# ipo-lab/lqp_py

Hardware: AMD Instinct MI355X
Metric: QPs/sec forward+backward, batch=128 dz=500 tol=1e-5 (higher is better)
Workload: dtype f32; 1 GPU; BASELINE configs[2]: batch=128/GPU dz=500 m=1 box+equality QP, ADMM forward + fixed-point backward, eps 1e-5, scale+adaptive_rho defaults; global_batch=128, seeds=10 batches, seeds 0..9 per rank, cycled, iters=60, checks=4, launch_mode=3, sync=False, linsolve=spd, loop_workgroups_per_qp=2, parallelism=batch-sharded x1, rccl_world_size=1

## Files before the change

lqp_py_amd/csrc/lqp_amd.hip:

```cpp
#include "../../include/lqp_amd.h"
#include "lqp_boxqp.hpp"
#include "lqp_unroll.hpp"
#ifdef LQP_SPLIT_BUILD
#include "split/lqp_extern.inc"
#endif

#include <cstdio>
#include <cstdlib>
#include <cstring>
#include <algorithm>
#include <atomic>
#include <chrono>
#include <mutex>
#include <vector>
#include <string>
#include <unordered_map>

using namespace lqp;

namespace {

constexpr int kRing = 2048;
inline int max_rows(int dtype) { return dtype == LQP_F32 ? 4096 : 2048; }
constexpr size_t kAlign = 256;
// ... 1179 lines not shown
    SoloScope one_wg_lu;
    for (;;) {
        const Knobs k = knobs();
        if (retry & 4) one_wg_lu.enter();
        FwdParams<T> P = L.P;
        FwdPlan<T> plan;
        int rc = plan_forward(P, ctl, retry, k, d, plan);
        if (rc) return rc;
        int n_launch = 0;
        rc = enqueue_prologue(st, P, plan, n_launch);
        if (rc) return rc;
        const Attempt a = plan.up_front ? run_planned(st, P, plan, ctl, stats, n_launch) : run_chunked(st, P, plan, ctl, stats, n_launch);
        switch (a.why) {
        case GU_NONE: return a.status;
        case GU_NOT_SPD: retry |= 1; break;
        case GU_LU_TIMEOUT: one_wg_lu.enter(); break;
        case GU_SEG_TIMEOUT: retry |= 2; break;
        case GU_SHARED_TIMEOUT: retry |= 4; break;
        }
    }
}

template <typename T>
size_t carve_backward(void* ws, int B, int n, int m, BwdParams<T>& P) {
    P.B = B; P.n = n; P.m = m; P.N = n + m;
    P.Np = round_up(P.N, LQP_NB); P.K = P.Np / LQP_NB;
    Carver c(ws);
    P.info = c.take<int>(B);
    P.piv = c.take<int>((size_t)B * P.Np);
    P.dest = c.take<int>((size_t)B * P.Np);
    P.rhs = c.take<T>((size_t)B * P.Np);
    P.rhs2 = c.take<T>((size_t)B * P.Np);
    P.bsc = c.take<T>((size_t)B * P.Np);
    P.fidx = c.take<int>((size_t)B * n);
    P.nred = c.take<int>(B);
    P.M = c.take<T>((size_t)B * P.Np * P.Np);
    P.packed = c.take<T>((size_t)B * packed_blocks(P.K) * LQP_BLK);
    return c.off + kAlign;
}

template <typename T>
int backward_impl(hipStream_t st, int B, int n, int m, const void* g, const void* x, const void* u, const void* lams,
                  const void* nus, const void* Q, const void* A, const void* lb, const void* ub, int rho_mode,
                  double rho_value, const void* rho_in, void* dQ, void* dp, void* dA, void* db, void* dlb, void* dub,
                  int32_t* fail_index, void* ws, size_t ws_bytes, int linsolve, void* host_report, const int kkt = 0,
                  int phase = 0) {
    const Knobs k = knobs();
    BwdParams<T> P;
    memset(&P, 0, sizeof(P));
    P.kkt = kkt ? 1 : 0;
    const bool reported = (linsolve & LQP_BWD_REPORTED) != 0;
    linsolve &= ~LQP_BWD_REPORTED;
    if (linsolve & LQP_BWD_PREFACTORED) { linsolve &= ~LQP_BWD_PREFACTORED; if (phase == 0 && !kkt) phase = 2; }
    P.host_report = (int*)host_report;
    bool reset_pending = P.host_report != nullptr;
    P.early_report = k.bwd_early != 0 ? 1 : 0;
    const size_t need = carve_backward<T>(ws, B, n, m, P);
    if (ws_bytes < need) return LQP_ERR_WORKSPACE;
    if (!k.bwd_equil) P.bsc = nullptr;
    P.g = (const T*)g; P.x = (const T*)x; P.u = (const T*)u; P.lams = (const T*)lams; P.nus = (const T*)nus;
    P.Q = (const T*)Q; P.A = (const T*)A; P.lb = (const T*)lb; P.ub = (const T*)ub; P.rho_in = (const T*)rho_in;
    P.rho_value = (T)rho_value; P.rho_mode = rho_mode;
    P.dQ = (T*)dQ; P.dp = (T*)dp; P.dA = (T*)dA; P.db = (T*)db; P.dlb = (T*)dlb; P.dub = (T*)dub;
    P.dbg = g_lu_dbg;
    P.reduced = (k.bwd_full && !kkt) ? 0 : 1;
    const int* nvec = P.reduced ? P.nred : nullptr;
    bool chol = false;
    if constexpr (sizeof(T) == 4) {
        chol = P.reduced && linsolve == 2 && k.bwd_chol && round_up(n, LQP_NB) / LQP_NB <= SPD_BIGK &&
               m <= SPD_MAXM && bwd_chol_lds_bytes(n, m, m >= 3 ? 4 : 2) <= 160 * 1024;
    }
    const bool lu_phases = !chol && P.reduced && !kkt;
    if (!chol && !lu_phases) {
        if (phase == 1) return LQP_ERR_UNSUPPORTED;
        phase = 0;
    }
    P.phase = phase;
    P.reported = (reported && phase == 2 && P.host_report && P.early_report) ? 1 : 0;
    if (reset_pending && !P.reported) report_reset(P.host_report, B);
    reset_pending = false;
    if constexpr (sizeof(T) == 4) {
        if (chol) {
            P.chol = 1;
            if (phase != 2) {
                const int lds = (2 * round_up(n, 8) + LQP_NW + 8 + round_up(n, 64) + 64) * 4;
                ProfScope ps(st, PC_BWD_BUILD);
                const int split = B <= 128 ? 2 : 1;
                hipLaunchKernelGGL(k_bwd_build_chol<>, dim3(B, split), dim3(LQP_NT), lds, st, P);
            }
            const bool nr4 = m >= 3;
            const int lds = bwd_chol_lds_bytes(n, m, nr4 ? 4 : 2);
            {
                const int Kmax = round_up(n, LQP_NB) / LQP_NB;
                P.la_maxk = !k.bwd_lookahead ? 0 : (Kmax < SPD_MAXK ? Kmax : SPD_MAXK - 1);
            }
            auto chol_fn = nr4 ? k_bwd_chol_solve<4> : k_bwd_chol_solve<0>;
#if LQP_PIV_MFMA
            if (k.spd_f16 != 0 && k.bwd_f16 != 0) chol_fn = nr4 ? k_bwd_chol_solve<4, true> : k_bwd_chol_solve<0, true>;
#endif
            int r2 = ensure_lds((const void*)chol_fn, lds);
            if (r2) return r2;
            ProfScope ps(st, PC_BWD_CHOL);
            hipLaunchKernelGGL(chol_fn, dim3(B), dim3(LQP_NT), lds, st, P);
            if (phase == 1) return hipGetLastError() == hipSuccess ? LQP_OK : LQP_ERR_HIP;
        }
    }
    if (chol) {
    } else if (phase == 2) {
        ProfScope ps(st, PC_BWD_BUILD);
        hipLaunchKernelGGL(k_bwd_gather_rhs<T>, dim3(B), dim3(256), 0, st, P);
    } else if (P.reduced) {
        const int lds = (round_up(n, 8) + LQP_NW + 8) * 4;
        ProfScope ps(st, PC_BWD_BUILD);
        const int split = (B <= 128 && k.split2) ? 2 : 1;
        hipLaunchKernelGGL(k_bwd_build_reduced<T>, dim3(B, split), dim3(LQP_NT), lds, st, P);
    } else {
        ProfScope ps(st, PC_BWD_BUILD);
        hipLaunchKernelGGL(k_bwd_build<T>, dim3(B), dim3(LQP_NT), 0, st, P);
    }
    int rc = LQP_OK;
    if (!chol) {
        if (phase != 2) {
            rc = launch_lu(st, P.M, B, P.N, P.Np, (size_t)P.Np * P.Np, P.piv, P.Np, P.info, nullptr, nvec,
                           (unsigned long long*)P.packed, packed_blocks(P.K) * LQP_BLK * sizeof(T) / 8);
            if (rc) return rc;
            if (P.host_report && (phase == 1 || (P.early_report && fail_index))) {
                ProfScope ps(st, PC_MISC);
                hipLaunchKernelGGL(k_report_info<>, dim3((B + 255) / 256), dim3(256), 0, st, (const int*)P.info, P.host_report, B);
                P.lu_reported = 1;
            }
            rc = launch_pack<T>(st, B, P.M, P.N, P.Np, (size_t)P.Np * P.Np, P.piv, P.Np, P.packed, P.dest, nullptr, nvec);
            if (rc) return rc;
            if (phase == 1) return hipGetLastError() == hipSuccess ? LQP_OK : LQP_ERR_HIP;
        } else if (P.reported) P.lu_reported = 1;
        rc = launch_solve<T>(st, B, P.packed, P.N, P.dest, P.rhs, 1, (size_t)P.Np, 1, 0, nvec);
        if (rc) return rc;
        if (P.reduced && !kkt && k.bwd_refine) {
            const int lds = (round_up(n, 8) + round_up(m > 0 ? m : 1, 8)) * (int)sizeof(T) + round_up(n, 8) * 4;
            { ProfScope ps(st, PC_BWD_BUILD);
              hipLaunchKernelGGL(k_bwd_residual<T>, dim3(B, (B <= 128 && k.split2) ? 2 : 1), dim3(LQP_NT), lds, st, P); }
            rc = launch_solve<T>(st, B, P.packed, P.N, P.dest, P.rhs2, 1, (size_t)P.Np, 1, 0, nvec);
            if (rc) return rc;
            P.refine = 1;
        }
    }
    {
        const int lds = (2 * n + m + 8) * (int)sizeof(T);
        auto fn = k_bwd_epilogue<T>;
        rc = ensure_lds((const void*)fn, lds);
        if (rc) return rc;
        ProfScope ps(st, PC_BWD_EPILOGUE);
        const int slabs = (k.epi_slabs < 0 ? (B <= 128 ? 2 : 1) : k.epi_slabs);
        hipLaunchKernelGGL(fn, dim3(B, slabs), dim3(LQP_NT), lds, st, P);
    }
    if (hipGetLastError() != hipSuccess) return LQP_ERR_HIP;
    if (fail_index) {
        int fi = -1;
        if (P.host_report && k.sync_plan != 0) {
            rc = wait_report(st, P.host_report, B);
            if (rc) return rc;
            bool gave_up = false;
            for (int i = 0; i < B; ++i) {
                const int v = ((const volatile int*)P.host_report)[i];
                if (v != 0 && fi < 0) fi = i;
                gave_up = gave_up || v == -7;
            }
            rc = gave_up ? LQP_ERR_TIMEOUT : fi >= 0 ? LQP_ERR_SINGULAR : LQP_OK;
        } else
            rc = first_failure(st, P.info, B, &fi, P.host_report);
        if (rc == LQP_ERR_TIMEOUT && !chol && !t_single_wg_lu) {
            SingleWgLu only;
            return backward_impl<T>(st, B, n, m, g, x, u, lams, nus, Q, A, lb, ub, rho_mode, rho_value, rho_in, dQ, dp, dA,
                                    db, dlb, dub, fail_index, ws, ws_bytes, 1, host_report, kkt, 0);
        }
        if (rc == LQP_ERR_SINGULAR && chol)
            return backward_impl<T>(st, B, n, m, g, x, u, lams, nus, Q, A, lb, ub, rho_mode, rho_value, rho_in, dQ, dp, dA,
                                    db, dlb, dub, fail_index, ws, ws_bytes, 1, host_report, kkt, 0);
        *fail_index = fi;
// ... 754 lines not shown
```

lqp_py_amd/csrc/lqp_boxqp.hpp:

```cpp
#pragma once
#include <type_traits>
#include "lqp_common.hpp"
#include "lqp_lu.hpp"
#include "lqp_lu_big.hpp"
#include "lqp_lu2.hpp"
#include "lqp_lu_wide.hpp"
#include "lqp_trsv.hpp"
#include "lqp_spd.hpp"

namespace lqp {

enum { ST_DONE = 0, ST_FINAL_ITER = 1, ST_GATE = 2, ST_NFACTOR = 3, ST_RHO_UPDATED = 4,
       ST_TIMEOUT = 5, ST_NCHECK = 6, ST_NOTSPD = 7,
       ST_VOTE = 8,
       ST_ANY_LB = 12, ST_ANY_UB = 13,
       ST_RESUME = 14,
       ST_WORDS = 16 };
enum { RP_LB = 1, RP_UB = 2, RP_TIMEOUT = 4, RP_NOTSPD = 8 };
enum { CT_NOTOPT = 0, CT_ARRIVE = 1, CT_WANTS = 2, CT_TRIG = 3, CT_WORDS = 4 };
template <typename T>
__device__ __forceinline__ void trace_check(unsigned int* __restrict__ vtrace, const int it, const int check_solved, const int ring,
                                            const T pri, const T dua) {
    if (!vtrace) return;
    const int c = it / check_solved;
// ... 2329 lines not shown
    const T* lb = P.lb + (size_t)b * n;
    const T* ub = P.ub + (size_t)b * n;
    const T* g = P.g + (size_t)b * n;
    const T* Q = P.Q + (size_t)b * n * n;
    const T* A = P.A ? P.A + (size_t)b * m * n : nullptr;
    T* M = P.M + (size_t)b * Np * Np;
    T* rhs = P.rhs + (size_t)b * Np;
    if (tid == 0 && blockIdx.y == 0) P.info[b] = 0;
    int nf = 0;
    for (int i0 = 0; i0 < n; i0 += LQP_NT) {
        const int i = i0 + tid;
        bool keep = false;
        if (i < n) {
            if (P.kkt) keep = true;
            else {
                const T sxu = x[i] + u[i];
                keep = !(sxu > ub[i] || sxu < lb[i]);
            }
        }
        const unsigned long long bal = __ballot(keep);
        const int before = __popcll(bal & ((1ull << lane) - 1ull));
        if (i0 > 0) __syncthreads();
        if (lane == 0) wtot[w] = __popcll(bal);
        __syncthreads();
        int base = nf;
#pragma unroll
        for (int ww = 0; ww < LQP_NW; ++ww) {
            const int c = wtot[ww];
            if (ww < w) base += c;
            nf += c;
        }
        if (keep) {
            fl[base + before] = i;
            if (blockIdx.y == 0) P.fidx[(size_t)b * n + base + before] = i;
        }
    }
    if (tid == 0 && blockIdx.y == 0) P.nred[b] = nf + m;
    __syncthreads();
    const int wy = blockIdx.y, ny = gridDim.y;
    constexpr int GQ = 8;
    for (int a0 = (w * ny + wy) * 2; a0 < nf; a0 += LQP_NW * ny * 2) {
        const int a1 = a0 + 1 < nf ? a0 + 1 : a0;
        const int i0 = fl[a0], i1 = fl[a1];
        const T* q0 = Q + (size_t)i0 * n;
        const T* q1 = Q + (size_t)i1 * n;
        const T dg0 = P.kkt ? kkt_weight(P, b, i0) : T(1e-8), dg1 = P.kkt ? kkt_weight(P, b, i1) : T(1e-8);
        for (int c0 = 0; c0 < nf; c0 += 64 * GQ) {
            T v0[GQ], v1[GQ];
#pragma unroll
            for (int q = 0; q < GQ; ++q) {
                const int c = c0 + lane + 64 * q;
                const int col = fl[c < nf ? c : nf - 1];
                v0[q] = q0[col];
                v1[q] = q1[col];
            }
#pragma unroll
            for (int q = 0; q < GQ; ++q) {
                const int c = c0 + lane + 64 * q;
                if (c < nf) {
                    M[(size_t)a0 * Np + c] = c == a0 ? v0[q] + dg0 : v0[q];
                    if (a1 != a0) M[(size_t)a1 * Np + c] = c == a1 ? v1[q] + dg1 : v1[q];
                }
            }
        }
        for (int r = lane; r < m; r += 64) {
            M[(size_t)a0 * Np + nf + r] = A[(size_t)r * n + i0];
            if (a1 != a0) M[(size_t)a1 * Np + nf + r] = A[(size_t)r * n + i1];
        }
        if (lane == 0 && P.g) { rhs[a0] = -g[i0]; if (a1 != a0) rhs[a1] = -g[i1]; }
    }
    for (int r = w * ny + wy; r < m; r += LQP_NW * ny) {
        T* mr = M + (size_t)(nf + r) * Np;
        for (int c = lane; c < nf; c += 64) mr[c] = A[(size_t)r * n + fl[c]];
        for (int c = lane; c < m; c += 64) mr[nf + c] = (c == r && !P.kkt) ? T(1e-8) : T(0);
        if (lane == 0) rhs[nf + r] = T(0);
    }
}

__device__ __forceinline__ float bwd_equil_scale(const float d) {
    if (!(d > 0.f) || !(d < 3.0e38f)) return 1.f;
    const int h = (int)((__float_as_uint(d) >> 23) & 0xFFu) - 127;
    return __uint_as_float((unsigned int)(127 - (h >> 1)) << 23);
}
template <int LQP_ANY = 0>
__global__ __launch_bounds__(LQP_NT) void k_bwd_build_chol(const BwdParams<float> P) {
    extern __shared__ __attribute__((aligned(32))) char smem[];
    const int b = blockIdx.x, n = P.n, m = P.m, Np = P.Np;
    const int tid = threadIdx.x, lane = tid & 63, w = tid >> 6;
    int* fl = (int*)smem;
    int* wtot = fl + round_up(n, 8);
    const float* x = P.x + (size_t)b * n;
    const float* u = P.u + (size_t)b * n;
    const float* lb = P.lb + (size_t)b * n;
    const float* ub = P.ub + (size_t)b * n;
    const float* g = P.g + (size_t)b * n;
    const float* Q = P.Q + (size_t)b * n * n;
    const float* A = P.A ? P.A + (size_t)b * m * n : nullptr;
    const int Kmax = round_up(n, LQP_NB) / LQP_NB, Npm = Kmax * LQP_NB;
    float* Ls = P.packed + (size_t)b * sym_blocks(Kmax) * LQP_BLK;
    float* AF = P.M + (size_t)b * Np * Np;
    float* rhs = P.rhs + (size_t)b * Np;
    if (tid == 0 && blockIdx.y == 0) P.info[b] = 0;
    float* wl = (float*)(wtot + LQP_NW + 8);
    bool keep = false;
    if (tid < n) {
        if (P.kkt) { keep = true; wl[tid] = kkt_weight(P, b, tid); }
        else {
            const float sxu = x[tid] + u[tid];
            keep = !(sxu > ub[tid] || sxu < lb[tid]);
        }
    }
    const unsigned long long bal = __ballot(keep);
    const int before = __popcll(bal & ((1ull << lane) - 1ull));
    if (lane == 0) wtot[w] = __popcll(bal);
    __syncthreads();
    int base = 0, nf = 0;
#pragma unroll
    for (int ww = 0; ww < LQP_NW; ++ww) {
        const int c = wtot[ww];
        if (ww < w) base += c;
        nf += c;
    }
    if (keep) {
        fl[base + before] = tid;
        if (blockIdx.y == 0) P.fidx[(size_t)b * n + base + before] = tid;
    }
    if (tid == 0 && blockIdx.y == 0) P.nred[b] = nf + m;
    __syncthreads();
    const int Kb = round_up(nf, LQP_NB) / LQP_NB;
    const int r = tid >> 4, c4 = (tid & 15) * 4;
    const int nblk = sym_blocks(Kb);
    float* const sl = wl + round_up(n, 8);
    for (int a = tid; a < Npm; a += LQP_NT) {
        float sv = 1.f;
        if (P.bsc && a < nf) sv = bwd_equil_scale(Q[(size_t)fl[a] * n + fl[a]] + (P.kkt ? wl[fl[a]] : 1e-8f));
        sl[a] = sv;
        if (P.bsc && blockIdx.y == 0) P.bsc[(size_t)b * Np + a] = sv;
    }
    __syncthreads();
    for (int t = blockIdx.y; t < nblk; t += gridDim.y) {
        int j = 0;
        while (sym_idx(j + 1, j + 1, Kb) <= t && j + 1 < Kb) ++j;
        const int i = j + (t - sym_idx(j, j, Kb));
        const int a = i * 64 + r;
        const bool rok = a < nf;
        const size_t rowoff = (size_t)fl[rok ? a : 0] * n;
        float q4[4];
#pragma unroll
        for (int e = 0; e < 4; ++e) {
            const int c = j * 64 + c4 + e;
            q4[e] = Q[rowoff + fl[c < nf ? c : 0]];
        }
        V4<float> v;
#pragma unroll
        for (int e = 0; e < 4; ++e) {
            const int c = j * 64 + c4 + e;
            float val = (a == c) ? 1.f : 0.f;
            if (rok && c < nf) val = ((q4[e] + (a == c ? (P.kkt ? wl[fl[a]] : 1e-8f) : 0.f)) * sl[a]) * sl[c];
            v.v[e] = val;
        }
        *(V4<float>*)(Ls + (size_t)t * LQP_BLK + tid * 4) = v;
    }
    if (blockIdx.y == 0) {
        if (P.phase != 1)
            for (int a = tid; a < Npm; a += LQP_NT) rhs[a] = a < nf ? -g[fl[a]] * sl[a] : 0.f;
        for (int q = 0; q < m; ++q)
            for (int a = tid; a < Npm; a += LQP_NT) AF[(size_t)q * Npm + a] = a < nf ? A[(size_t)q * n + fl[a]] * sl[a] : 0.f;
    }
}

__host__ __device__ inline int bwd_chol_lds_bytes(int n, int m, int nr = 2) {
    const int Kmax = round_up(n, LQP_NB) / LQP_NB, Npm = Kmax * LQP_NB;
    const int a0 = spd_lds_bytes(Kmax > SPD_MAXK ? SPD_MAXK : Kmax);
    const int a = (Kmax < SPD_MAXK && chol_la_lds_bytes(Kmax) > a0) ? chol_la_lds_bytes(Kmax) : a0;
    const int c = ((1 + nr + m) * Npm + nr * 64 + nr * LQP_NW * 64 + m * m + 2 * m + 8) * 4;
    return a > c ? a : c;
}
template <int NRV = 0, bool F16 = false>
__global__ __launch_bounds__(LQP_NT) void k_bwd_chol_solve(const BwdParams<float> P) {
    extern __shared__ __attribute__((aligned(32))) char smem[];
    const int b = blockIdx.x, n = P.n, m = P.m, Np = P.Np;
    const int tid = threadIdx.x, lane = tid & 63, w = tid >> 6;
    const int Kmax = round_up(n, LQP_NB) / LQP_NB, Npm = Kmax * LQP_NB;
    const int nf = P.nred[b] - m;
    const int Kb = round_up(nf, LQP_NB) / LQP_NB, Nb = Kb * LQP_NB;
    float* Ls = P.packed + (size_t)b * sym_blocks(Kmax) * LQP_BLK;
    const float* AF = P.M + (size_t)b * Np * Np;
    float* rhs = P.rhs + (size_t)b * Np;
    unsigned long long dt0 = P.dbg ? clock64() : 0;
    if (Kb > 0 && P.phase != 2) {
        if (Kb <= P.la_maxk) wg_chol_factor_la<F16>(Ls, Kb, P.info + b, smem, P.dbg ? P.dbg + (size_t)b * 8 : nullptr);
        else if (Kb <= SPD_MAXK) wg_chol_factor(Ls, Kb, P.info + b, smem);
        else wg_chol_factor_big(Ls, Kb, P.info + b, smem);
    }
    if (P.host_report && (P.early_report || P.phase == 1) && !P.reported) {
        __syncthreads();
        if (tid == 0)
            __hip_atomic_store(P.host_report + b, __hip_atomic_load(P.info + b, __ATOMIC_RELAXED, __HIP_MEMORY_SCOPE_AGENT),
                               __ATOMIC_RELAXED, __HIP_MEMORY_SCOPE_SYSTEM);
    }
    if (P.phase == 1) return;
    __syncthreads();
    if (P.dbg && tid == 0) { const unsigned long long t = clock64(); P.dbg[(size_t)b * 8 + 0] = t - dt0; dt0 = t; P.dbg[(size_t)b * 8 + 3] = Kb; }
    constexpr int NR = NRV == 4 ? 4 : 2;
    float* acc = (float*)smem;
    float* u0 = acc + (size_t)NR * Npm;
    float* G = u0 + Npm;
    float* t = G + (size_t)m * Npm;
    float* part = t + NR * 64;
    float* S = part + NR * LQP_NW * 64;
    float* wv = S + m * m;
    float* dn = wv + m;
    if (P.phase == 2) {
        const float* g = P.g + (size_t)b * n;
        const int* fidx = P.fidx + (size_t)b * n;
        const float* bs_ = P.bsc ? P.bsc + (size_t)b * Np : nullptr;
        for (int e = tid; e < Nb; e += LQP_NT) u0[e] = e < nf ? -g[fidx[e]] * (bs_ ? bs_[e] : 1.f) : 0.f;
    } else {
        for (int e = tid; e < Nb; e += LQP_NT) u0[e] = rhs[e];
    }
    for (int q = 0; q < m; ++q)
        for (int e = tid; e < Nb; e += LQP_NT) G[(size_t)q * Npm + e] = AF[(size_t)q * Npm + e];
    __syncthreads();
    if (Kb > 0)
        for (int c0 = 0; c0 < 1 + m; c0 += NR)
            wg_chol_solve_n<NR>(Ls, Kb, u0 + (size_t)c0 * Npm, Npm, (1 + m - c0) < NR ? (1 + m - c0) : NR, acc, t, part,
                                (P.dbg && P.la_maxk == 0) ? P.dbg + (size_t)b * 8 : nullptr);
    if (P.dbg && tid == 0) { const unsigned long long t = clock64(); P.dbg[(size_t)b * 8 + 1] = t - dt0; dt0 = t; }
    if (m > 0) {
        for (int e = w; e < m * m + m; e += LQP_NW) {
            const int q = e < m * m ? e / m : e - m * m;
            const float* rv = e < m * m ? G + (size_t)(e - q * m) * Npm : u0;
            float a = 0.f;
            for (int i = lane; i < nf; i += 64) a += AF[(size_t)q * Npm + i] * rv[i];
            a = wave_sum(a);
            if (lane == 0) {
                if (e < m * m) S[e] = a - ((e / m == e % m) ? 1e-8f : 0.f);
                else wv[q] = a;
            }
        }
        __syncthreads();
        {
            const int rr = tid / (m + 1), jj = tid - rr * (m + 1);
            const bool mine = tid < m * (m + 1);
            int* pivrow = (int*)dn;
            for (int c = 0; c < m; ++c) {
                if (tid == 0) {
                    int pr = c;
                    float best = tabs(S[c * m + c]);
                    for (int r2 = c + 1; r2 < m; ++r2) if (tabs(S[r2 * m + c]) > best) { best = tabs(S[r2 * m + c]); pr = r2; }
                    const bool skip = !(best > 0.f);
                    if (skip && P.info[b] == 0) P.info[b] = nf + c + 1;
                    pivrow[0] = pr; pivrow[1] = skip ? 1 : 0;
                }
                __syncthreads();
                const int pr = pivrow[0];
                const bool skip = pivrow[1] != 0;
                float* const rowc = jj < m ? S + c * m + jj : wv + c;
                float* const rowp = jj < m ? S + pr * m + jj : wv + pr;
                float* const rowr = jj < m ? S + rr * m + jj : wv + rr;
                if (!skip && pr != c && tid <= m) {
                    const float tmp = *rowc; *rowc = *rowp; *rowp = tmp;
                }
                __syncthreads();
                const float inv = skip ? 0.f : 1.f / S[c * m + c];
                const float f = (mine && !skip) ? S[rr * m + c] : 0.f;
                __syncthreads();
                if (!skip && tid <= m) *rowc *= inv;
                __syncthreads();
                if (mine && !skip && rr != c) *rowr -= f * *rowc;
                __syncthreads();
            }
            for (int q = tid; q < m; q += LQP_NT) dn[q] = wv[q];
        }
        __syncthreads();
// ... 293 lines not shown
```

lqp_py_amd/csrc/lqp_spd.hpp:

```cpp
#pragma once
#include "lqp_common.hpp"
#include "lqp_lu.hpp"
#include "lqp_trsv.hpp"
#include "lqp_f16x2.hpp"

namespace lqp {

constexpr int SPD_LS = 68;
constexpr int SPD_MAXK = 8;
constexpr int SPD_MAXM = 16;

__host__ __device__ constexpr int sym_blocks(int K) { return K * (K + 1) / 2; }
__host__ __device__ constexpr int sym_idx(int i, int j, int K) { return j * K - j * (j - 1) / 2 + (i - j); }
#ifndef LQP_PIV_WAVES
#define LQP_PIV_WAVES 16
#endif
#ifndef LQP_PIV_WAVES_RS
#define LQP_PIV_WAVES_RS 8
#endif
#ifndef LQP_PIV_NB
#define LQP_PIV_NB 4
#endif
constexpr int PIV_NB = LQP_PIV_NB;
constexpr int PIV_LDS = 2 * PIV_NB * 64 + 64;
// ... 2570 lines not shown
            }
            for (int u = 0; u < cn; ++u)
                *(V4<float>*)(Hs + (size_t)sym_idx(k + 1 + c0 + u, k, K) * LQP_BLK + tid * 4) =
                    *(const V4<float>*)(Y + ((size_t)u * 64 + r) * SPD_LS + cq * 4);
            __syncthreads();
        }
        __threadfence_block();
        __syncthreads();
        const int ng = (np + BIG_G - 1) / BIG_G;
        for (int ga = 0; ga < ng; ++ga) {
            for (int gb = 0; gb <= ga; ++gb) {
                const int a0 = BIG_G * ga, b0 = BIG_G * gb;
                const int an = (np - a0) < BIG_G ? (np - a0) : BIG_G, bn = (np - b0) < BIG_G ? (np - b0) : BIG_G;
                const int boff = gb == ga ? 0 : BIG_G;
                for (int u = 0; u < an; ++u)
                    *(V4<float>*)(Y + ((size_t)u * 64 + r) * SPD_LS + cq * 4) =
                        *(const V4<float>*)(Hs + (size_t)sym_idx(k + 1 + a0 + u, k, K) * LQP_BLK + tid * 4);
                if (gb != ga)
                    for (int u = 0; u < bn; ++u)
                        *(V4<float>*)(Y + ((size_t)(BIG_G + u) * 64 + r) * SPD_LS + cq * 4) =
                            *(const V4<float>*)(Hs + (size_t)sym_idx(k + 1 + b0 + u, k, K) * LQP_BLK + tid * 4);
                __syncthreads();
                const int npair = gb == ga ? an * (an + 1) / 2 : an * bn;
                auto decode = [&](const int task, int& ua, int& ub, bool& skip, bool& mirror) -> float* {
                    const int qi = (task >> 1) & 1, qj = task & 1, p = task >> 2;
                    if (gb == ga) {
                        ua = 0;
                        while ((ua + 1) * (ua + 2) / 2 <= p) ++ua;
                        ub = p - ua * (ua + 1) / 2;
                    } else {
                        ua = p / bn;
                        ub = p - ua * bn;
                    }
                    const int si = a0 + ua, sj = b0 + ub;
                    skip = si == sj && qi == 0 && qj == 1;
                    mirror = si == sj && qi == 1 && qj == 0;
                    return Hs + (size_t)sym_idx(k + 1 + si, k + 1 + sj, K) * LQP_BLK;
                };
                auto load_c = [&](const float* T0, const int task, f32x16& c) {
                    const float* C = T0 + (32 * ((task >> 1) & 1)) * 64 + 32 * (task & 1) + li;
#pragma unroll
                    for (int q = 0; q < 16; ++q) c[q] = C[quad_row(q, lh) * 64];
                };
                const int ntask = npair * 4;
                int task = __builtin_amdgcn_readfirstlane(w);
                int ua = 0, ub = 0; bool skip = false, mirror = false;
                float* T0 = nullptr;
                f32x16 nxt;
                if (task < ntask) { T0 = decode(task, ua, ub, skip, mirror); if (!skip) load_c(T0, task, nxt); }
                while (task < ntask) {
                    const int qi = (task >> 1) & 1, qj = task & 1;
                    f32x16 cur = nxt;
                    float* Tc = T0;
                    const int cua = ua, cub = ub;
                    const bool cskip = skip, cmirror = mirror;
                    const int nt = task + LQP_NW;
                    if (nt < ntask) { T0 = decode(nt, ua, ub, skip, mirror); if (!skip) load_c(T0, nt, nxt); }
                    if (!cskip) {
                        const f32x16 acc = spd_quadrant(Y + ((size_t)cua * 64 + 32 * qi) * SPD_LS,
                                                        Y + ((size_t)(boff + cub) * 64 + 32 * qj) * SPD_LS);
                        cur -= acc;
                        float* C = Tc + (32 * qi) * 64 + 32 * qj + li;
#pragma unroll
                        for (int q = 0; q < 16; ++q) C[quad_row(q, lh) * 64] = cur[q];
                        if (cmirror) {
#pragma unroll
                            for (int q = 0; q < 16; ++q) Tc[li * 64 + 32 + quad_row(q, lh)] = cur[q];
                        }
                    }
                    task = nt;
                }
                __syncthreads();
            }
        }
        __threadfence_block();
        __syncthreads();
    }
    if (tid == 0 && flag[0] != 0 && *info == 0) *info = flag[0];
}

constexpr int CHOL_LA_CHAIN = 4;
__host__ __device__ inline int chol_la_lds_bytes(int K) { return spd_lds_bytes(K) + 64 + 64 * 64 * 4; }

template <bool F16 = false>
__device__ __forceinline__ void wg_chol_factor_la(float* __restrict__ Hs, const int K, int* __restrict__ info, char* smem,
                                                  unsigned long long* __restrict__ dbg = nullptr) {
    constexpr int NCH = CHOL_LA_CHAIN, NTW = LQP_NW - NCH, NTT = NTW * 64;
    const int tid = threadIdx.x, lane = tid & 63, w = tid >> 6;
    const int li = lane & 31, lh = lane >> 5;
    const int nslot = K > 1 ? K - 1 : 1;
    float* Y = (float*)smem;
    float* W = Y + (size_t)nslot * 64 * SPD_LS;
    float* WT = W + 64 * SPD_LS;
    float* pcol = WT + 64 * SPD_LS;
    int* flag = (int*)(pcol + PIV_LDS);
    int* sy = flag + 4;
    float* St = (float*)(flag + 20);
    if (tid < 20) flag[tid] = 0;
    *(V4<float>*)(St + tid * 4) = *(const V4<float>*)(Hs + (size_t)sym_idx(0, 0, K) * LQP_BLK + tid * 4);
    __syncthreads();
    if (w < NCH) {
        __builtin_amdgcn_s_setprio(3);
        int gt = 0;
        for (int k = 0; k < K; ++k) {
            unsigned long long c0 = dbg ? clock64() : 0;
            lds_wait_ge(sy + 2, 3 * k);
            lds_wait_ge(sy + 4, k);
            if (dbg && tid == 0) { const unsigned long long c1 = clock64(); dbg[4] += c1 - c0; c0 = c1; }
#if LQP_PIV_MFMA
            wg_pivot_block_mfma<true, true, false, F16>(St, W, WT, pcol, flag, k * 64, sy + 5, k, 0.f, false, pcol + 128);
#else
            wg_pivot_block<NCH, true>(St, W, WT, pcol, flag, k * 64, sy + 0, &gt);
#endif
            lds_group_sync<true>(sy + 0, gt += NCH);
            if (tid == 0) __hip_atomic_store(sy + 3, k + 1, __ATOMIC_RELAXED, __HIP_MEMORY_SCOPE_WORKGROUP);
            for (int v = tid; v < 1024; v += NCH * 64)
                *(V4<float>*)(Hs + (size_t)sym_idx(k, k, K) * LQP_BLK + v * 4) = *(const V4<float>*)(W + (v >> 4) * SPD_LS + (v & 15) * 4);
            if (dbg && tid == 0) dbg[5] += clock64() - c0;
        }
        __builtin_amdgcn_s_setprio(0);
    } else {
        const int tw = w - NCH, tt = tid - NCH * 64;
        int gt = 0;
        for (int k = 0; k < K; ++k) {
            const int np = K - 1 - k;
            for (int s = 0; s < np; ++s) {
                const float* src = Hs + (size_t)sym_idx(k + 1 + s, k, K) * LQP_BLK;
                for (int v = tt; v < 1024; v += NTT)
                    *(V4<float>*)(Y + ((size_t)s * 64 + (v >> 4)) * SPD_LS + (v & 15) * 4) = *(const V4<float>*)(src + v * 4);
            }
            const int nupd = np * (np + 1) / 2 * 4;
            f32x16 pre;
            if (tw < nupd && !(tw == 1)) {
                const int qi = (tw >> 1) & 1, qj = tw & 1, p = tw >> 2;
                int si = 0;
                while ((si + 1) * (si + 2) / 2 <= p) ++si;
                const int sj = p - si * (si + 1) / 2;
                if (!(si == sj && qi == 0 && qj == 1)) {
                    const float* C = Hs + (size_t)sym_idx(k + 1 + si, k + 1 + sj, K) * LQP_BLK + (32 * qi) * 64 + 32 * qj + li;
#pragma unroll
                    for (int q = 0; q < 16; ++q) pre[q] = C[quad_row(q, lh) * 64];
                }
            }
            lds_group_sync(sy + 1, gt += NTW);
            unsigned long long c0 = dbg ? clock64() : 0;
            lds_wait_ge(sy + 3, k + 1);
            if (dbg && tt == 0) { const unsigned long long c1 = clock64(); dbg[6] += c1 - c0; c0 = c1; }
            [[maybe_unused]] float* const ysc = pcol + 144;
            [[maybe_unused]] char* const Yc = (char*)Y;
            [[maybe_unused]] const int lane_b = li * F2_ROW + 32 * lh;
            if constexpr (F16) {
                float sW, isW;
                f2_scale_of(tmax((pcol + 128)[1], (pcol + 128)[2]), sW, isW);
                for (int task = tw; task < np * 2; task += NTW) {
                    const int s = task >> 1, qi = task & 1;
                    const float* prow = Y + ((size_t)s * 64 + 32 * qi + li) * SPD_LS;
                    float pv[4][8], mx = 0.f;
#pragma unroll
                    for (int c = 0; c < 4; ++c) {
                        f2_load_cell_f32(prow, c, lh, pv[c]);
#pragma unroll
                        for (int j = 0; j < 8; ++j) mx = tmax(mx, tabs(pv[c][j]));
                    }
                    mx = wave_max(mx);
                    float sP, isP;
                    f2_scale_of(mx, sP, isP);
                    F2Cell pb[4];
#pragma unroll
                    for (int c = 0; c < 4; ++c) {
#pragma unroll
                        for (int j = 0; j < 8; ++j) pv[c][j] *= sP;
                        f2_split8(pv[c], pb[c].hi, pb[c].mid);
                    }
                    f32x16 a0, a1;
#pragma unroll
                    for (int q = 0; q < 16; ++q) { a0[q] = 0.f; a1[q] = 0.f; }
#pragma unroll
                    for (int c = 0; c < 4; ++c) {
                        float wv[8];
                        F2Cell wc;
                        if (c < 2) {
                            f2_load_cell_f32(W + li * SPD_LS, c, lh, wv);
#pragma unroll
                            for (int j = 0; j < 8; ++j) wv[j] *= sW;
                            f2_split8(wv, wc.hi, wc.mid);
                            a0 = f2_mma(wc, pb[c], a0);
                        }
                        f2_load_cell_f32(W + (32 + li) * SPD_LS, c, lh, wv);
#pragma unroll
                        for (int j = 0; j < 8; ++j) wv[j] *= sW;
                        f2_split8(wv, wc.hi, wc.mid);
                        a1 = f2_mma(wc, pb[c], a1);
                    }
                    const float un = isW * isP;
                    if (lane == 0) ysc[task] = un * 2097152.f;
                    float* dstg = Hs + (size_t)sym_idx(k + 1 + s, k, K) * LQP_BLK + (32 * qi + li) * 64 + 4 * lh;
                    char* dstl = Yc + ((size_t)s * 64 + 32 * qi) * F2_ROW + lane_b;
#pragma unroll
                    for (int hsel = 0; hsel < 2; ++hsel) {
#pragma unroll
                        for (int c = 0; c < 2; ++c) {
                            float v[8];
#pragma unroll
                            for (int gq = 0; gq < 2; ++gq) {
                                V4<float> o;
#pragma unroll
                                for (int e = 0; e < 4; ++e) {
                                    const float a = hsel ? a1[8 * c + 4 * gq + e] : a0[8 * c + 4 * gq + e];
                                    o.v[e] = a * un;
                                    v[4 * gq + e] = a * 4.76837158203125e-7f;
                                }
                                *(V4<float>*)(dstg + 32 * hsel + 8 * (2 * c + gq)) = o;
                            }
                            h16x8 hi, mid;
                            f2_split8(v, hi, mid);
                            f2_write_cell(dstl + 64 * (2 * hsel + c), hi, mid);
                        }
                    }
                }
            } else {
            for (int task = tw; task < np * 2; task += NTW) {
                const int s = task >> 1, qi = task & 1;
                float* Xp = Y + ((size_t)s * 64 + 32 * qi) * SPD_LS;
                const f32x16 a0 = spd_quadrant<1, false>(Xp, W);
                const f32x16 a1 = spd_quadrant(Xp, W + 32 * SPD_LS);
#pragma unroll
                for (int q = 0; q < 16; ++q) {
// ... 190 lines not shown
```

Measured before the change: 198,800 QPs/sec.

## Fuse backward Cholesky matrix gather into look-ahead factorization kernel

```diff
diff --git a/lqp_py_amd/csrc/lqp_amd.hip b/lqp_py_amd/csrc/lqp_amd.hip
--- a/lqp_py_amd/csrc/lqp_amd.hip
+++ b/lqp_py_amd/csrc/lqp_amd.hip
@@ -1285,6 +1285,10 @@
     if constexpr (sizeof(T) == 4) {
         if (chol) {
             P.chol = 1;
+            {
+                const int Kmax = round_up(n, LQP_NB) / LQP_NB;
+                P.la_maxk = !k.bwd_lookahead ? 0 : (Kmax < SPD_MAXK ? Kmax : SPD_MAXK - 1);
+            }
             if (phase != 2) {
                 const int lds = (2 * round_up(n, 8) + LQP_NW + 8 + round_up(n, 64) + 64) * 4;
                 ProfScope ps(st, PC_BWD_BUILD);
@@ -1293,10 +1297,6 @@
             }
             const bool nr4 = m >= 3;
             const int lds = bwd_chol_lds_bytes(n, m, nr4 ? 4 : 2);
-            {
-                const int Kmax = round_up(n, LQP_NB) / LQP_NB;
-                P.la_maxk = !k.bwd_lookahead ? 0 : (Kmax < SPD_MAXK ? Kmax : SPD_MAXK - 1);
-            }
             auto chol_fn = nr4 ? k_bwd_chol_solve<4> : k_bwd_chol_solve<0>;
 #if LQP_PIV_MFMA
             if (k.spd_f16 != 0 && k.bwd_f16 != 0) chol_fn = nr4 ? k_bwd_chol_solve<4, true> : k_bwd_chol_solve<0, true>;
diff --git a/lqp_py_amd/csrc/lqp_boxqp.hpp b/lqp_py_amd/csrc/lqp_boxqp.hpp
--- a/lqp_py_amd/csrc/lqp_boxqp.hpp
+++ b/lqp_py_amd/csrc/lqp_boxqp.hpp
@@ -2435,6 +2435,27 @@
     const int h = (int)((__float_as_uint(d) >> 23) & 0xFFu) - 127;
     return __uint_as_float((unsigned int)(127 - (h >> 1)) << 23);
 }
+__device__ __forceinline__ bool gather_in_chol(const BwdParams<float>& P, const int Kb) {
+    return Kb > 0 && Kb <= P.la_maxk && P.phase != 2;
+}
+__device__ __forceinline__ float bwd_block_entry(const float q, const int a, const int c, const int nf, const float dg,
+                                                 const float sa, const float sc) {
+    float val = (a == c) ? 1.f : 0.f;
+    if (a < nf && c < nf) val = ((q + (a == c ? dg : 0.f)) * sa) * sc;
+    return val;
+}
+struct BwdBlockSource {
+    const BwdParams<float>& P;
+    const int b;
+    const float* Q;
+    const int* idx;
+    const float* sc;
+    int n, nf;
+    __device__ __forceinline__ float diag(const int i) const { return P.kkt ? kkt_weight(P, b, i) : 1e-8f; }
+    __device__ __forceinline__ float entry(const float q, const int a, const int c, const float dg, const float sa, const float sc_) const {
+        return bwd_block_entry(q, a, c, nf, dg, sa, sc_);
+    }
+};
 template <int LQP_ANY = 0>
 __global__ __launch_bounds__(LQP_NT) void k_bwd_build_chol(const BwdParams<float> P) {
     extern __shared__ __attribute__((aligned(32))) char smem[];
@@ -2481,16 +2502,26 @@
     if (tid == 0 && blockIdx.y == 0) P.nred[b] = nf + m;
     __syncthreads();
     const int Kb = round_up(nf, LQP_NB) / LQP_NB;
+    const bool in_chol = gather_in_chol(P, Kb);
+    if (in_chol && blockIdx.y != 0) return;
+    float* const sl = wl + round_up(n, 8);
+    for (int a = tid; a < Npm; a += LQP_NT) {
+        const int ia = nf > 0 ? fl[a < nf ? a : nf - 1] : 0;
+        const float qd = Q[(size_t)ia * n + ia];
+        float sv = 1.f;
+        if (P.bsc && a < nf) sv = bwd_equil_scale(qd + (P.kkt ? wl[ia] : 1e-8f));
+        sl[a] = sv;
+        if (blockIdx.y == 0) {
+            if (P.bsc) P.bsc[(size_t)b * Np + a] = sv;
+            if (P.phase != 1)
+                rhs[a] = a < nf ? -g[ia] * sv : 0.f;
+            for (int q = 0; q < m; ++q) AF[(size_t)q * Npm + a] = a < nf ? A[(size_t)q * n + ia] * sv : 0.f;
+        }
+    }
+    if (in_chol) return;
+    __syncthreads();
     const int r = tid >> 4, c4 = (tid & 15) * 4;
     const int nblk = sym_blocks(Kb);
-    float* const sl = wl + round_up(n, 8);
-    for (int a = tid; a < Npm; a += LQP_NT) {
-        float sv = 1.f;
-        if (P.bsc && a < nf) sv = bwd_equil_scale(Q[(size_t)fl[a] * n + fl[a]] + (P.kkt ? wl[fl[a]] : 1e-8f));
-        sl[a] = sv;
-        if (P.bsc && blockIdx.y == 0) P.bsc[(size_t)b * Np + a] = sv;
-    }
-    __syncthreads();
     for (int t = blockIdx.y; t < nblk; t += gridDim.y) {
         int j = 0;
         while (sym_idx(j + 1, j + 1, Kb) <= t && j + 1 < Kb) ++j;
@@ -2508,17 +2539,9 @@
 #pragma unroll
         for (int e = 0; e < 4; ++e) {
             const int c = j * 64 + c4 + e;
-            float val = (a == c) ? 1.f : 0.f;
-            if (rok && c < nf) val = ((q4[e] + (a == c ? (P.kkt ? wl[fl[a]] : 1e-8f) : 0.f)) * sl[a]) * sl[c];
-            v.v[e] = val;
+            v.v[e] = bwd_block_entry(q4[e], a, c, nf, P.kkt ? wl[fl[rok ? a : 0]] : 1e-8f, sl[a], sl[c]);
         }
         *(V4<float>*)(Ls + (size_t)t * LQP_BLK + tid * 4) = v;
-    }
-    if (blockIdx.y == 0) {
-        if (P.phase != 1)
-            for (int a = tid; a < Npm; a += LQP_NT) rhs[a] = a < nf ? -g[fl[a]] * sl[a] : 0.f;
-        for (int q = 0; q < m; ++q)
-            for (int a = tid; a < Npm; a += LQP_NT) AF[(size_t)q * Npm + a] = a < nf ? A[(size_t)q * n + fl[a]] * sl[a] : 0.f;
     }
 }
 
@@ -2542,8 +2565,11 @@
     float* rhs = P.rhs + (size_t)b * Np;
     unsigned long long dt0 = P.dbg ? clock64() : 0;
     if (Kb > 0 && P.phase != 2) {
-        if (Kb <= P.la_maxk) wg_chol_factor_la<F16>(Ls, Kb, P.info + b, smem, P.dbg ? P.dbg + (size_t)b * 8 : nullptr);
-        else if (Kb <= SPD_MAXK) wg_chol_factor(Ls, Kb, P.info + b, smem);
+        if (gather_in_chol(P, Kb)) {
+            const BwdBlockSource src{P, b, P.Q + (size_t)b * n * n, P.fidx + (size_t)b * n, P.bsc ? P.bsc + (size_t)b * Np : nullptr, n, nf};
+            wg_chol_factor_la<F16>(Ls, Kb, P.info + b, smem, src, bwd_chol_lds_bytes(n, m, NRV == 4 ? 4 : 2),
+                                   P.dbg ? P.dbg + (size_t)b * 8 : nullptr);
+        } else if (Kb <= SPD_MAXK) wg_chol_factor(Ls, Kb, P.info + b, smem);
         else wg_chol_factor_big(Ls, Kb, P.info + b, smem);
     }
     if (P.host_report && (P.early_report || P.phase == 1) && !P.reported) {
diff --git a/lqp_py_amd/csrc/lqp_spd.hpp b/lqp_py_amd/csrc/lqp_spd.hpp
--- a/lqp_py_amd/csrc/lqp_spd.hpp
+++ b/lqp_py_amd/csrc/lqp_spd.hpp
@@ -2676,8 +2676,9 @@
 constexpr int CHOL_LA_CHAIN = 4;
 __host__ __device__ inline int chol_la_lds_bytes(int K) { return spd_lds_bytes(K) + 64 + 64 * 64 * 4; }
 
-template <bool F16 = false>
+template <bool F16 = false, class Src>
 __device__ __forceinline__ void wg_chol_factor_la(float* __restrict__ Hs, const int K, int* __restrict__ info, char* smem,
+                                                  const Src& src, const int lds_bytes,
                                                   unsigned long long* __restrict__ dbg = nullptr) {
     constexpr int NCH = CHOL_LA_CHAIN, NTW = LQP_NW - NCH, NTT = NTW * 64;
     const int tid = threadIdx.x, lane = tid & 63, w = tid >> 6;
@@ -2691,7 +2692,39 @@
     int* sy = flag + 4;
     float* St = (float*)(flag + 20);
     if (tid < 20) flag[tid] = 0;
-    *(V4<float>*)(St + tid * 4) = *(const V4<float>*)(Hs + (size_t)sym_idx(0, 0, K) * LQP_BLK + tid * 4);
+    int* const fl_l = (int*)(St + 64 * 64);
+    float* const sl_l = (float*)(fl_l + K * 64);
+    const bool in_lds = chol_la_lds_bytes(K) + K * 64 * 8 <= lds_bytes;
+    const int nf = src.nf;
+    {
+        const int a = tid >> 4, c0 = (tid & 15) * 4;
+        const unsigned int ia = src.idx[a < nf ? a : 0];
+        unsigned int ic[4];
+        float scv[4], q[4];
+#pragma unroll
+        for (int e = 0; e < 4; ++e) ic[e] = src.idx[c0 + e < nf ? c0 + e : 0];
+#pragma unroll
+        for (int e = 0; e < 4; ++e) q[e] = *(const float*)((const char*)src.Q + (size_t)((ia * (unsigned int)src.n + ic[e]) * 4u));
+        const bool scaled = src.sc != nullptr;
+        const float* const scp = scaled ? src.sc : src.Q;
+        float sa = scp[a < nf ? a : 0];
+#pragma unroll
+        for (int e = 0; e < 4; ++e) scv[e] = scp[c0 + e < nf ? c0 + e : 0];
+        if (!scaled) {
+            sa = 1.f;
+#pragma unroll
+            for (int e = 0; e < 4; ++e) scv[e] = 1.f;
+        }
+        const float dg = (a >> 2) == (c0 >> 2) ? src.diag((int)ia) : 0.f;
+        V4<float> v;
+#pragma unroll
+        for (int e = 0; e < 4; ++e) v.v[e] = src.entry(q[e], a, c0 + e, dg, sa, scv[e]);
+        *(V4<float>*)(St + tid * 4) = v;
+        if (in_lds && tid < K * 64) {
+            fl_l[tid] = src.idx[tid < nf ? tid : 0];
+            sl_l[tid] = src.sc ? src.sc[tid] : 1.f;
+        }
+    }
     __syncthreads();
     if (w < NCH) {
         __builtin_amdgcn_s_setprio(3);
@@ -2716,27 +2749,92 @@
     } else {
         const int tw = w - NCH, tt = tid - NCH * 64;
         int gt = 0;
+        auto gather_rest = [&](const int* __restrict__ fl, const float* __restrict__ sl) __attribute__((always_inline)) {
+            constexpr int GQ = 4, RT = NTT / 16;
+            const int c4 = (tt & 15) * 4;
+            const int total = (K - 1) * 64 + K * (K - 1) * 32;
+            const bool scaled = sl != nullptr;
+            const float* const slp = scaled ? sl : src.Q;
+            for (int u0 = tt >> 4; u0 < total; u0 += GQ * RT) {
+                int ra[GQ], rr[GQ], rj[GQ];
+#pragma unroll
+                for (int t = 0; t < GQ; ++t) {
+                    const int u = u0 + t * RT;
+                    int j = 0, rem = u, nr = (K - 1) * 64;
+#pragma unroll
+                    for (int s = 0; s < SPD_MAXK - 2; ++s) {
+                        const bool adv = rem >= nr && j < K - 1;
+                        rem -= adv ? nr : 0;
+                        j += adv ? 1 : 0;
+                        nr = (K - j) * 64;
+                    }
+                    rj[t] = u < total ? j : -1;
+                    rr[t] = rem;
+                    ra[t] = u < total ? (j == 0 ? 64 : j * 64) + rem : 0;
+                }
+                unsigned int ia[GQ], ic[GQ][4];
+#pragma unroll
+                for (int t = 0; t < GQ; ++t) {
+                    const int cb = (rj[t] < 0 ? 0 : rj[t]) * 64 + c4;
+                    ia[t] = fl[ra[t] < nf ? ra[t] : 0];
+#pragma unroll
+                    for (int e = 0; e < 4; ++e) ic[t][e] = fl[cb + e < nf ? cb + e : 0];
+                }
+                float q[GQ][4], sa[GQ], sc[GQ][4];
+#pragma unroll
+                for (int t = 0; t < GQ; ++t)
+#pragma unroll
+                    for (int e = 0; e < 4; ++e) q[t][e] = *(const float*)((const char*)src.Q + (size_t)((ia[t] * (unsigned int)src.n + ic[t][e]) * 4u));
+#pragma unroll
+                for (int t = 0; t < GQ; ++t) {
+                    const int cb = (rj[t] < 0 ? 0 : rj[t]) * 64 + c4;
+                    sa[t] = slp[ra[t] < nf ? ra[t] : 0];
+#pragma unroll
+                    for (int e = 0; e < 4; ++e) sc[t][e] = slp[cb + e < nf ? cb + e : 0];
+                }
+#pragma unroll
+                for (int t = 0; t < GQ; ++t) {
+                    if (rj[t] >= 0) {
+                        const int j = rj[t], a = ra[t], cb = j * 64 + c4;
+                        const float dg = (a >> 2) == (cb >> 2) ? src.diag(fl[a < nf ? a : 0]) : 0.f;
+                        V4<float> v;
+#pragma unroll
+                        for (int e = 0; e < 4; ++e)
+                            v.v[e] = src.entry(q[t][e], a, cb + e, dg, scaled ? sa[t] : 1.f, scaled ? sc[t][e] : 1.f);
+                        if (j == 0) *(V4<float>*)(Y + (size_t)rr[t] * SPD_LS + c4) = v;
+                        else *(V4<float>*)(Hs + (size_t)sym_idx(j, j, K) * LQP_BLK + rr[t] * 64 + c4) = v;
+                    }
+                }
+            }
+        };
+        if (in_lds) gather_rest(fl_l, sl_l);
+        else gather_rest(src.idx, src.sc);
         for (int k = 0; k < K; ++k) {
             const int np = K - 1 - k;
-            for (int s = 0; s < np; ++s) {
-                const float* src = Hs + (size_t)sym_idx(k + 1 + s, k, K) * LQP_BLK;
-                for (int v = tt; v < 1024; v += NTT)
-                    *(V4<float>*)(Y + ((size_t)s * 64 + (v >> 4)) * SPD_LS + (v & 15) * 4) = *(const V4<float>*)(src + v * 4);
-            }
+            if (k > 0)
+                for (int s = 0; s < np; ++s) {
+                    const float* blk = Hs + (size_t)sym_idx(k + 1 + s, k, K) * LQP_BLK;
+                    for (int v = tt; v < 1024; v += NTT)
+                        *(V4<float>*)(Y + ((size_t)s * 64 + (v >> 4)) * SPD_LS + (v & 15) * 4) = *(const V4<float>*)(blk + v * 4);
+                }
             const int nupd = np * (np + 1) / 2 * 4;
             f32x16 pre;
-            if (tw < nupd && !(tw == 1)) {
-                const int qi = (tw >> 1) & 1, qj = tw & 1, p = tw >> 2;
-                int si = 0;
-                while ((si + 1) * (si + 2) / 2 <= p) ++si;
-                const int sj = p - si * (si + 1) / 2;
-                if (!(si == sj && qi == 0 && qj == 1)) {
-                    const float* C = Hs + (size_t)sym_idx(k + 1 + si, k + 1 + sj, K) * LQP_BLK + (32 * qi) * 64 + 32 * qj + li;
-#pragma unroll
-                    for (int q = 0; q < 16; ++q) pre[q] = C[quad_row(q, lh) * 64];
-                }
-            }
+            auto fetch_pre = [&]() __attribute__((always_inline)) {
+                if (tw < nupd && !(tw == 1)) {
+                    const int qi = (tw >> 1) & 1, qj = tw & 1, p = tw >> 2;
+                    int si = 0;
+                    while ((si + 1) * (si + 2) / 2 <= p) ++si;
+                    const int sj = p - si * (si + 1) / 2;
+                    if (!(si == sj && qi == 0 && qj == 1)) {
+                        const float* C = Hs + (size_t)sym_idx(k + 1 + si, k + 1 + sj, K) * LQP_BLK + (32 * qi) * 64 + 32 * qj + li;
+#pragma unroll
+                        for (int q = 0; q < 16; ++q) pre[q] = C[quad_row(q, lh) * 64];
+                    }
+                }
+            };
+            if (k > 0) fetch_pre();
             lds_group_sync(sy + 1, gt += NTW);
+            if (k == 0) fetch_pre();
             unsigned long long c0 = dbg ? clock64() : 0;
             lds_wait_ge(sy + 3, k + 1);
             if (dbg && tt == 0) { const unsigned long long c1 = clock64(); dbg[6] += c1 - c0; c0 = c1; }
```

Measured after the change: 194,900 QPs/sec. -1.9%, worse.
